# cboin1996/avddpg

Hardware: AMD Instinct MI355X
Metric: env-steps/sec + DDPG updates/sec, 4096x5-vehicle platoons (higher is better)
Workload: dtype f32-class (fp16 hi+lo operand pairs on the 16-bit matrix cores, f32 accumulate)

## Files before the change

### avddpg_amd/csrc/fsplit.hip

```cpp
#include <type_traits>

#include "fset_common.h"
#include "anchor.h"
#include "smooth.h"

namespace avd {
namespace fsplit {
using namespace fset;

struct ActorS {
    static constexpr int K = 256, KP = 256, NFT = 8, NKS = 16, LD = 264, NGT = 9, KG = 288;
    static constexpr bool critic = false;
};
struct CriticS {
    static constexpr int K = 304, KP = 320, NFT = 10, NKS = 19, LD = 312, NGT = 10, KG = 320;
    static constexpr bool critic = true;
};
constexpr int NGT_MAX = 10;

template <int I, int N, class F>
__device__ __forceinline__ void static_for(F&& f) {
    if constexpr (I < N) {
        f(std::integral_constant<int, I>{});
        static_for<I + 1, N>(f);
// ... 19 lines not shown
    f32x2 l;
#ifdef __HIP_DEVICE_COMPILE__
    asm("v_fma_mix_f32 %0, -%1, 1.0, %2 op_sel:[0,0,0] op_sel_hi:[1,0,0]" : "=v"(l[0]) : "v"(hi), "v"(a));
    asm("v_fma_mix_f32 %0, -%1, 1.0, %2 op_sel:[1,0,0] op_sel_hi:[1,0,0]" : "=v"(l[1]) : "v"(hi), "v"(b));
#else
    l[0] = a - (float)h[0], l[1] = b - (float)h[1];
#endif
    lo = __builtin_bit_cast(unsigned, __builtin_convertvector(l, f16x2));
}
__device__ __forceinline__ void split1h(float x, f16& hi, f16& lo) {
    hi = (f16)x;
    lo = (f16)(x - (float)hi);
}
template <class V>
__device__ __forceinline__ void pin16(V& x) {
#pragma unroll
    for (int q = 0; q < 2; ++q) {
        float a = x[8 * q], b = x[8 * q + 1], c = x[8 * q + 2], d = x[8 * q + 3], e = x[8 * q + 4], f = x[8 * q + 5], g = x[8 * q + 6], h = x[8 * q + 7];
        asm volatile("" : "+v"(a), "+v"(b), "+v"(c), "+v"(d), "+v"(e), "+v"(f), "+v"(g), "+v"(h));
        x[8 * q] = a, x[8 * q + 1] = b, x[8 * q + 2] = c, x[8 * q + 3] = d, x[8 * q + 4] = e, x[8 * q + 5] = f, x[8 * q + 6] = g, x[8 * q + 7] = h;
    }
}
__device__ __forceinline__ f16x8 fragh(unsigned a, unsigned b, unsigned c, unsigned d) {
    uint4 o;
    o.x = a, o.y = b, o.z = c, o.w = d;
    return __builtin_bit_cast(f16x8, o);
}
__device__ __forceinline__ f32x16 mfmah(f16x8 a, f16x8 b, f32x16 c) {
    return __builtin_amdgcn_mfma_f32_32x32x16_f16(a, b, c, 0, 0, 0);
}
__device__ __forceinline__ f16x8 make_xh(float x0, float x1, float x2, float x3, int h) {
    f16 a0, a1, a2, a3, l0, l1, l2, l3;
    split1h(x0, a0, l0), split1h(x1, a1, l1), split1h(x2, a2, l2), split1h(x3, a3, l3);
    const f16 one = (f16)1.f, zero = (f16)0.f;
    f16x8 v;
    v[0] = a0, v[1] = a1, v[2] = a2, v[3] = a3;
    v[4] = h ? one : l0, v[5] = h ? one : l1, v[6] = h ? zero : l2, v[7] = h ? zero : l3;
    return v;
}
__device__ __forceinline__ f16x8 make_wh(float w0, float w1, float w2, float w3, float b, float sc, int h) {
    f16 a0, a1, a2, a3, l0, l1, l2, l3, bh, bl;
    split1h(sc * w0, a0, l0), split1h(sc * w1, a1, l1), split1h(sc * w2, a2, l2), split1h(sc * w3, a3, l3), split1h(sc * b, bh, bl);
    const f16 zero = (f16)0.f;
    f16x8 v;
    v[0] = h ? l0 : a0, v[1] = h ? l1 : a1, v[2] = h ? l2 : a2, v[3] = h ? l3 : a3;
    v[4] = h ? bh : a0, v[5] = h ? bl : a1, v[6] = h ? bh : a2, v[7] = h ? zero : a3;
    return v;
}
__device__ __forceinline__ f16x8 make_xg(float x0, float x1, float x2, float x3, float g, int h) {
    f16 a0, a1, a2, a3, l0, l1, l2, l3, gh, gl;
    split1h(x0, a0, l0), split1h(x1, a1, l1), split1h(x2, a2, l2), split1h(x3, a3, l3), split1h(g, gh, gl);
    const f16 zero = (f16)0.f;
    f16x8 v;
    v[0] = a0, v[1] = a1, v[2] = a2, v[3] = a3;
    v[4] = h ? gh : l0, v[5] = h ? gh : l1, v[6] = h ? gl : l2, v[7] = h ? zero : l3;
    return v;
}

template <int S>
__device__ __forceinline__ void load_x(const float* xa, long row, float (&x)[4]) {
    if (S == 4) {
        const float4 v = *(const float4*)(xa + 4 * row);
        x[0] = v.x, x[1] = v.y, x[2] = v.z, x[3] = v.w;
    } else {
#pragma unroll
        for (int k = 0; k < 4; ++k) x[k] = k < S ? xa[S * row + k] : 0.f;
    }
}

__host__ __device__ constexpr int wpos(int f) { return (f & ~12) | ((f & 4) << 1) | ((f & 8) >> 1); }

struct NetP {
    const float* th;
    long th_stride;
    const f16* Whi;
    const f16* Wlo;
    const f16* Wchi;
    const f16* Wclo;
    const f16x8* wf1h;
    const float* vec;
    const unsigned* wap;
};

struct PackArgs {
    const float* x[2];
    const float* extra[2];
    f16x8* outh[2];
    long rows;
};
__device__ __forceinline__ void front_flag(unsigned* wave_flags, bool hit) {
    const bool any = __ballot(hit) != 0;
    if ((threadIdx.x & 63) == 0) wave_flags[threadIdx.x >> 6] = any;
}
template <int S>
__device__ __forceinline__ void pack_x_role(const PackArgs& a, int which, long bx, unsigned* wave_flags) {
    const float* x = a.x[which];
    const float* extra = a.extra[which];
    const bool extra_is_action = which == 0;
    const long i = bx * 256 + threadIdx.x;
    bool nf = false;
    if (i < 2 * a.rows) {
        float v[4];
        load_x<S>(x, i >> 1, v);
        nf = not_finite(v[0]) || not_finite(v[1]) || not_finite(v[2]) || not_finite(v[3]);
        nf = nf || fmaxf(fmaxf(fabsf(v[0]), fabsf(v[1])), fmaxf(fabsf(v[2]), fabsf(v[3]))) >= F16_OVERFLOW;
        if (!(i & 1)) {
            const float e = extra[i >> 1];
            nf = nf || not_finite(e) || (extra_is_action && fabsf(e) >= F16_OVERFLOW);
        }
        a.outh[which][i] = make_xh(v[0], v[1], v[2], v[3], (int)(i & 1));
    }
    front_flag(wave_flags, nf);
}

struct PrepArgs {
    avd_mlp_layout L;
    int S;
    const float *theta, *stats, *theta_t, *stats_t;
    f16 *Whi[4], *Wlo[4];
    f16 *Wchi[4], *Wclo[4];
    f16x8* wf1h[4];
    float* vec[4];
    unsigned* wap;
    unsigned* smax;
    int* bad;
    unsigned* fflag;
    int n_fflag;
};
constexpr int SCALE_SLICES = 16;
__device__ __forceinline__ float pow2_for(float mx) {
    int e = 0;
    if (mx > 0.f && !not_finite(mx)) (void)frexpf(mx, &e);
    int k = 13 - e;
    k = k < -14 ? -14 : (k > 30 ? 30 : k);
    return ldexpf(1.f, k);
}
__device__ __forceinline__ void scale_role(const PrepArgs& a, int net, int set, int slice, int n_sets) {
    __shared__ float red[256], red2[256], c3a[H2], inva[CriticS::K];
    const int tid = threadIdx.x;
    const bool critic = net & 1, target = net >= 2;
    const avd_mlp_layout& L = a.L;
    const float* th = (target ? a.theta_t : a.theta) + (long)set * L.theta_size + (critic ? L.actor_size : 0);
    const float* st = (target ? a.stats_t : a.stats) + (long)set * L.stats_size;
    const int K = critic ? CriticS::K : ActorS::K, oW2 = critic ? L.cW2 : L.aW2;
    const int og2 = critic ? L.cg3 : L.ag2, omv2 = critic ? L.cmv3 : L.amv2, oW3 = critic ? L.cW3 : L.aW3;
    if (tid < H2) c3a[tid] = fabsf((1.0f / sqrtf(st[omv2 + tid] + BN_EPS)) * th[og2 + tid] * th[oW3 + tid]);
    for (int f = tid; f < K; f += 256) {
        int og, omv, ff = f;
        if (!critic) og = L.ag1, omv = L.amv1;
        else if (f < H1) og = L.cgs, omv = L.cmvs;
        else og = L.cga, omv = L.cmva, ff = f - H1;
        inva[f] = fabsf((1.0f / sqrtf(st[omv + ff] + BN_EPS)) * th[og + ff]);
    }
    __syncthreads();
    const int total = K * H2, per = (total + SCALE_SLICES - 1) / SCALE_SLICES, lo = slice * per, hi = min(total, lo + per);
    float m = 0.f, m2 = 0.f;
    for (int i = lo + tid; i < hi; i += 256) {
        const float w = fabsf(th[oW2 + i]);
        m = fmaxf(m, inva[i / H2] * w);
        m2 = fmaxf(m2, c3a[i % H2] * w);
    }
    red[tid] = m, red2[tid] = m2;
    __syncthreads();
    for (int o = 128; o > 0; o >>= 1) {
        if (tid < o) red[tid] = fmaxf(red[tid], red[tid + o]), red2[tid] = fmaxf(red2[tid], red2[tid + o]);
        __syncthreads();
    }
    if (tid == 0) {
        unsigned* dst = a.smax + (((long)net * n_sets + set) * SCALE_SLICES + slice) * 2;
        dst[0] = __float_as_uint(red[0]);
        dst[1] = __float_as_uint(red2[0]);
    }
}
__global__ __launch_bounds__(320) void prep_kernel(const PrepArgs a) {
    __shared__ float red[320];
    const int n = blockIdx.x, net = blockIdx.y, set = blockIdx.z, f = threadIdx.x;
    const bool critic = net & 1, target = net >= 2;
    const avd_mlp_layout& L = a.L;
    const float* th = (target ? a.theta_t : a.theta) + (long)set * L.theta_size + (critic ? L.actor_size : 0);
    const float* st = (target ? a.stats_t : a.stats) + (long)set * L.stats_size;
    const int K = critic ? CriticS::K : ActorS::K, KP = critic ? CriticS::KP : ActorS::KP;
    const int oW2 = critic ? L.cW2 : L.aW2, ob2 = critic ? L.cb2 : L.ab2, oW3 = critic ? L.cW3 : L.aW3, ob3 = critic ? L.cb3 : L.ab3;
    const int og2 = critic ? L.cg3 : L.ag2, obe2 = critic ? L.cbe3 : L.abe2, omm2 = critic ? L.cmm3 : L.amm2, omv2 = critic ? L.cmv3 : L.amv2;
    const float inv2n = (1.0f / sqrtf(st[omv2 + n] + BN_EPS)) * th[og2 + n], c3n = inv2n * th[oW3 + n];
    const unsigned* smax = a.smax + ((long)net * gridDim.z + set) * SCALE_SLICES * 2;
    unsigned mx = 0, mxc = 0;
#pragma unroll
    for (int sl = 0; sl < SCALE_SLICES; ++sl) mx = max(mx, smax[2 * sl]), mxc = max(mxc, smax[2 * sl + 1]);
    const float SW = pow2_for(__uint_as_float(mx)), SWC = pow2_for(__uint_as_float(mxc));
    if (net == 0 && set == 0) {
        unsigned any = 0;
        for (int w0 = n * 320 + f; w0 < a.n_fflag; w0 += 4 * H2 * 320) {
            unsigned v[4];
#pragma unroll
            for (int u = 0; u < 4; ++u) v[u] = a.fflag[min(w0 + u * H2 * 320, a.n_fflag - 1)];
// ... 23 lines not shown
            a.Whi[net][at] = hi, a.Wlo[net][at] = lo;
        }
        if (!target) {
            f16 hi, lo;
            const float wc = SWC * (c3n * w);
            if (fabsf(wc) >= F16_OVERFLOW) atomicOr(a.bad, 1);
            split1h(wc, hi, lo);
            const long at = ((long)set * KP + f) * H2 + n;
            a.Wchi[net][at] = hi, a.Wclo[net][at] = lo;
        }
    }
    red[f] = shw;
    __syncthreads();
    if (f < 64) red[f] += red[f + 256];
    __syncthreads();
    for (int o = 128; o > 0; o >>= 1) {
        if (f < o) red[f] += red[f + o];
        __syncthreads();
    }
    float* vec = a.vec[net] + (long)set * VEC;
    if (f == 0) {
        if (n == 0) vec[2 * H2 + 1] = SW, vec[2 * H2 + 2] = SWC;
        vec[n] = th[ob2 + n] + red[0];
        vec[H2 + n] = c3n;
        if (not_finite(vec[n]) || not_finite(c3n) || not_finite(th[ob3])) atomicOr(a.bad, 1);
    }
    if (n == 0) {
        __syncthreads();
        float v = 0.f;
        if (f < H2) {
            const float inv2 = (1.0f / sqrtf(st[omv2 + f] + BN_EPS)) * th[og2 + f];
            v = (th[obe2 + f] - st[omm2 + f] * inv2) * th[oW3 + f];
        }
        red[f] = v;
        __syncthreads();
        for (int o = 64; o > 0; o >>= 1) {
            if (f < o) red[f] += red[f + o];
            __syncthreads();
        }
        if (f == 0) vec[2 * H2] = th[ob3] + red[0];
    }
}
__device__ __forceinline__ bool prep1_role(const PrepArgs& a, int ft, int net, int set, int lane) {
    const int r = lane & 31, h = lane >> 5;
    bool hit = false;
    const bool critic = net & 1, target = net >= 2;
    const avd_mlp_layout& L = a.L;
    const float* th = (target ? a.theta_t : a.theta) + (long)set * L.theta_size + (critic ? L.actor_size : 0);
    const int K = critic ? CriticS::K : ActorS::K;
    const int f = 32 * ft + r;
    float w[4] = {0.f, 0.f, 0.f, 0.f}, b = 0.f;
    if (f == K) {
        b = 1.f;
    } else if (f < K) {
        if (critic && ft >= 8) {
            w[0] = th[L.cWa + (f - H1)], b = th[L.cba + (f - H1)];
        } else {
            const float* W = th + (critic ? L.cWs : L.aW1);
#pragma unroll
            for (int k = 0; k < 4; ++k) w[k] = k < a.S ? W[k * H1 + f] : 0.f;
            b = th[(critic ? L.cbs : L.ab1) + f];
        }
        if (not_finite(w[0]) || not_finite(w[1]) || not_finite(w[2]) || not_finite(w[3]) || not_finite(b)) hit = true;
        if (S1 * fmaxf(fmaxf(fabsf(w[0]), fabsf(w[1])), fmaxf(fmaxf(fabsf(w[2]), fabsf(w[3])), fabsf(b))) >= F16_OVERFLOW) hit = true;
    }
    a.wf1h[net][((long)set * NGT_MAX + ft) * 64 + lane] = make_wh(w[0], w[1], w[2], w[3], b, S1, h);
    if (net == 1 && ft == 0 && lane < 48) {
        const int hl = lane / 24, hh = (lane / 12) & 1, ks = (lane / 4) % 3, m = lane & 3;
        unsigned v = 0;
#pragma unroll
        for (int e = 0; e < 2; ++e) {
            const int jj = 2 * m + e, fa = 16 * ks + 8 * (jj >> 2) + 4 * hh + (jj & 3);
            f16 hi, lo;
            split1h(S1 * th[L.cWa + fa], hi, lo);
            v |= (unsigned)__builtin_bit_cast(unsigned short, hl ? lo : hi) << (16 * e);
        }
        a.wap[(long)set * 48 + lane] = v;
    }
    return hit;
}

struct FrontArgs {
    PrepArgs pa;
    PackArgs pk;
    float* grads;
    long n_grads;
    int n_sets, n_scale, n_prep1, n_zero, n_pack;
};
constexpr int ZERO_PER_BLOCK = 4096;
template <int S>
__global__ __launch_bounds__(256) void front_kernel(const FrontArgs a) {
    int b = blockIdx.x;
    if (b < a.n_scale) {
        scale_role(a.pa, b & 3, (b >> 2) % a.n_sets, (b >> 2) / a.n_sets, a.n_sets);
        return;
    }
    b -= a.n_scale;
    if (b < a.n_prep1) {
        const int q = 4 * b + (threadIdx.x >> 6);
        bool hit = false;
        if (q < NGT_MAX * 4 * a.n_sets) hit = prep1_role(a.pa, q % NGT_MAX, (q / NGT_MAX) & 3, q / (NGT_MAX * 4), threadIdx.x & 63);
        front_flag(a.pa.fflag + 4 * (long)b, hit);
        return;
    }
    b -= a.n_prep1;
    if (b < a.n_zero) {
        if (b == 0 && threadIdx.x == 0) *a.pa.bad = 0;
        const long base = (long)b * ZERO_PER_BLOCK + threadIdx.x;
#pragma unroll
        for (int k = 0; k < ZERO_PER_BLOCK / 256; ++k)
            if (base + 256 * k < a.n_grads) a.grads[base + 256 * k] = 0.f;
        return;
    }
    b -= a.n_zero;
    const int which = b >= a.n_pack;
    pack_x_role<S>(a.pk, which, b - which * a.n_pack, a.pa.fflag + 4 * ((long)a.n_prep1 + b));
}

enum HeadMode { OUT_TANH = 0, OUT_TD = 1, HEAD_BOTH = 5, OUT_TANH_SAVE = 6 };
struct HeadArgs {
    unsigned long long* stamp;
    NetP net;
    int n_agents, n_sets;
    const f16x8* xf;
    const float* act;
    const float* act2;
    const float* r;
    const float* yin;
    const float* aw;
    float* out;
    unsigned* sm;
    float* g3;
    float* dmu;
    float* part_s;
    float* part_s2;
    float* part_m;
    float* tz;
    float gamma, high, inv_n;
    int* bad;
    int abl;
};
#ifndef HEAD_FAST
#define HEAD_FAST 5
#define HEAD_SLOW 3
#endif

template <int S, class NET, int MODE, bool HP = false, class... H>
__global__ __launch_bounds__(NT) void head_kernel(const HeadArgs p, H... hp) {
    constexpr int K = NET::K, NKS = NET::NKS, NFT = NET::NFT, LD = NET::LD;
    constexpr int NTH = NT;
    constexpr bool BOTH = (MODE == HEAD_BOTH);
    static_assert(!BOTH || NET::critic, "HEAD_BOTH is a critic mode");
    __shared__ __attribute__((aligned(16))) f16 wimg[2][H2 * LD];
    __shared__ __attribute__((aligned(16))) float b2s[H2];
    __shared__ __attribute__((aligned(16))) float c3s[H2];
    __shared__ __attribute__((aligned(16))) unsigned waps[BOTH ? 48 : 4];
    const int tid = threadIdx.x, w = tid >> 6, lane = tid & 63, r = lane & 31, h = lane >> 5, q = w >> 1, rh = w & 1;
    const int set = blockIdx.x % p.n_sets, j0 = blockIdx.x / p.n_sets, J = gridDim.x / p.n_sets, P = p.n_agents / p.n_sets;
#ifdef AVD_STAMP
    unsigned long long hacc[4] = {0, 0, 0, 0}, hlast = __builtin_amdgcn_s_memtime();
    const unsigned long long hstart = hlast;
#define HSTAMP(i) { const unsigned long long t_ = __builtin_amdgcn_s_memtime(); hacc[i] += t_ - hlast; hlast = t_; }
#else
#define HSTAMP(i)
#endif
    const float* vec = p.net.vec + (long)set * VEC;
    const f16x8* wf1 = p.net.wf1h + (long)set * NGT_MAX * 64 + lane;
    const f32x16 zero16 = {};
    const int ntile = j0 < P ? (P - j0 + J - 1) / J : 0;
    const int row = 32 * rh + r;
    f16x8 nx = {};
    float na = 0.f, nb = 0.f, ny = 0.f, nw = 1.f;
    auto fetch_in = [&](int k) {
        const int agent = (j0 + k * J) * p.n_sets + set;
        const long ri = (long)agent * TILE + row;
        nx = p.xf[2 * ri + h];
        if (NET::critic) na = p.act[ri];
        if (BOTH) nb = p.act2[ri];
        if (MODE == OUT_TD) ny = p.r[ri];
        if (BOTH) ny = p.yin[ri];
        if (BOTH && p.aw) nw = p.aw[agent];
    };
    constexpr int FAST = HEAD_FAST, SLOW = HEAD_SLOW, PERIOD = 2 * (FAST + SLOW);
    const int qs = __builtin_amdgcn_readfirstlane(q);
    const int cnt = qs < 2 ? FAST : SLOW, start = qs < 2 ? qs * FAST : 2 * FAST + (qs - 2) * SLOW;
    int k = start, pos = 0;
    auto next_tile = [&](int kk, int pp) { return pp + 1 == cnt ? kk + PERIOD - cnt + 1 : kk + 1; };
    const float SW = vec[2 * H2 + 1], d3 = vec[2 * H2];
    const float vb = vec[tid & (H2 - 1)], vc = vec[H2 + (tid & (H2 - 1))];
    unsigned wv = 0;
    if constexpr (BOTH) wv = p.net.wap[(long)set * 48 + (tid < 48 ? tid : 47)];
    f16x8 warm0 = wf1[0], warm1 = wf1[64];
    if (k < ntile) fetch_in(k);
    constexpr int PER = H2 * (K / 8), NLD = 2 * PER / NTH;
    static_assert(2 * PER % NTH == 0, "the image is a whole number of chunks per thread");
    typedef unsigned u32x4 __attribute__((ext_vector_type(4)));
    u32x4 img[NLD];
    static_for<0, NLD>([&](auto u_c) {
        constexpr int u = decltype(u_c)::value;
        const int i = tid + u * NTH, hl = i / PER, rem = i - hl * PER;
        img[u] = *(const u32x4*)((hl ? p.net.Wlo : p.net.Whi) + (long)set * H2 * K + 8 * rem);
    });
    __builtin_amdgcn_sched_barrier(0);
    const float sc = SW * S1, isc = 1.f / sc;
    if (tid < H2) b2s[tid] = vb * sc, c3s[tid] = vc * isc;
    if (BOTH && tid < 48) waps[tid] = wv;
    static_for<0, NLD>([&](auto u_c) {
        constexpr int u = decltype(u_c)::value;
        const int i = tid + u * NTH, hl = i / PER, rem = i - hl * PER, n = rem / (K / 8), c = rem - n * (K / 8);
        *(u32x4*)(&wimg[hl][n * LD + 8 * c]) = img[u];
    });
    asm volatile("" ::"v"(warm0), "v"(warm1));
    float Dacc = 0.f, Lacc = 0.f, Dacc2 = 0.f, Lacc2 = 0.f, gmax = 0.f;
    unsigned watch = 0;
    auto look = [&](float x) {
        unsigned u = __float_as_uint(x);
        asm volatile("" : "+v"(u));
        u &= 0x7fffffffu;
        watch = watch > u ? watch : u;
    };
    __syncthreads();

    const f16* whi0 = &wimg[0][r * LD + 8 * h];
    const f16* wlo0 = &wimg[1][r * LD + 8 * h];
    constexpr int NSEQ = BOTH ? 8 : NFT;
    HSTAMP(3);
    for (int ui = 0; k < ntile; ++ui, k = next_tile(k, pos), pos = pos + 1 == cnt ? 0 : pos + 1) {
        const int agent = (j0 + k * J) * p.n_sets + set;
        const long ri = (long)agent * TILE + row;
        const f16x8 xs = nx, xa = make_xh(na, 0.f, 0.f, 0.f, h), xb = BOTH ? make_xh(nb, 0.f, 0.f, 0.f, h) : xa;
        const float ty = ny, tw = nw;
        if (next_tile(k, pos) < ntile) fetch_in(next_tile(k, pos));
        f32x16 acc[4];
#pragma unroll
        for (int t = 0; t < 4; ++t)
#pragma unroll
            for (int g = 0; g < 4; ++g) {
                const float4 b = *(const float4*)(b2s + 32 * t + 8 * g + 4 * h);
                acc[t][4 * g] = b.x, acc[t][4 * g + 1] = b.y, acc[t][4 * g + 2] = b.z, acc[t][4 * g + 3] = b.w;
            }
        unsigned ph[8], pl[8];
        auto split16 = [&](const f32x16& p1) {
            if (FSPLIT_ABL(p.abl) & 4) {
#pragma unroll
                for (int m = 0; m < 8; ++m) ph[m] = __float_as_uint(p1[2 * m]), pl[m] = __float_as_uint(p1[2 * m + 1]);
                return;
            }
#pragma unroll
            for (int m = 0; m < 8; ++m) split2h(relu(p1[2 * m]), relu(p1[2 * m + 1]), ph[m], pl[m]);
        };
        auto zdot_t = [&](f32x16& a, int t) {
            float zp = 0.f;
#pragma unroll
            for (int g = 0; g < 4; ++g) {
                const float4 c = *(const float4*)(c3s + 32 * t + 8 * g + 4 * h);
                const float cc[4] = {c.x, c.y, c.z, c.w};
#pragma unroll
                for (int j = 0; j < 4; ++j) {
                    a[4 * g + j] = relu(a[4 * g + j]);
                    zp = fmaf(a[4 * g + j], cc[j], zp);
                }
            }
            return zp;
        };
        auto zdot_nd = [&](const f32x16& a, int t) {
            float zp = 0.f;
#pragma unroll
            for (int g = 0; g < 4; ++g) {
                const float4 c = *(const float4*)(c3s + 32 * t + 8 * g + 4 * h);
                const float cc[4] = {c.x, c.y, c.z, c.w};
#pragma unroll
                for (int j = 0; j < 4; ++j) zp = fmaf(relu(a[4 * g + j]), cc[j], zp);
            }
            return zp;
        };
        auto mask_t = [&](const f32x16& a) {
            unsigned b = 0;
#pragma unroll
            for (int g = 0; g < 4; ++g)
#pragma unroll
                for (int j = 0; j < 4; ++j) b |= a[4 * g + j] > 0.f ? 1u << (4 * g + (j >> 1) + 16 * (j & 1)) : 0u;
            return b;
        };
        auto mask_store = [&](const unsigned (&b)[4], unsigned* dst) {
            const auto s0 = __builtin_amdgcn_permlane32_swap(b[0], b[2], false, false);
            const auto s1 = __builtin_amdgcn_permlane32_swap(b[1], b[3], false, false);
            uint2 o;
            o.x = s0[0] | (s0[1] << 2), o.y = s1[0] | (s1[1] << 2);
            *(uint2*)(dst + 2 * h) = o;
        };
        auto out_z = [&](f32x16 (&ac)[4]) {
            float zp = 0.f;
#pragma unroll
            for (int t = 0; t < 4; ++t) zp += zdot_t(ac[t], t);
            zp += __shfl_xor(zp, 32);
            return d3 + zp;
        };
        split16(mfmah(wf1[0], xs, zero16));
        f16x8 wfn = wf1[64];
        f16x8 wg[2][2][2];
        auto read_group = [&](int g, f16x8 (&dst)[2][2]) {
            const int ks = g >> 1, th = g & 1;
#pragma unroll
            for (int tt = 0; tt < 2; ++tt) {
                dst[tt][0] = *(const f16x8*)(whi0 + 32 * (2 * th + tt) * LD + 16 * ks);
                dst[tt][1] = *(const f16x8*)(wlo0 + 32 * (2 * th + tt) * LD + 16 * ks);
            }
        };
        read_group(0, wg[0]);
        auto tile = [&](auto si_c, f32x16 (&ac)[4]) {
            constexpr int si = decltype(si_c)::value;
            constexpr int ft = si;
            f32x16 p1n = zero16;
            if constexpr (si + 1 < NSEQ) {
                p1n = mfmah(wfn, (NET::critic && si + 1 >= 8) ? xa : xs, zero16);
                if constexpr (si + 2 < NSEQ) wfn = wf1[64 * (si + 2)];
            }
#pragma unroll
            for (int s = 0; s < 2; ++s) {
                const int ks = 2 * ft + s;
                if (ks >= NKS) continue;
                const f16x8 bhi = fragh(ph[4 * s], ph[4 * s + 1], ph[4 * s + 2], ph[4 * s + 3]);
                const f16x8 blo = fragh(pl[4 * s], pl[4 * s + 1], pl[4 * s + 2], pl[4 * s + 3]);
#pragma unroll
                for (int th = 0; th < 2; ++th) {
                    const int g = 2 * ks + th;
                    if (g + 1 < 2 * (BOTH ? 16 : NKS)) read_group(g + 1, wg[(g + 1) & 1]);
#pragma unroll
                    for (int tt = 0; tt < 2; ++tt) {
                        const int t = 2 * th + tt;
                        const f16x8 whi = wg[g & 1][tt][0], wlo = wg[g & 1][tt][1];
                        ac[t] = mfmah(whi, bhi, ac[t]);
                        ac[t] = mfmah(wlo, bhi, ac[t]);
                        ac[t] = mfmah(whi, blo, ac[t]);
                    }
                }
            }
            if constexpr (si + 1 < NSEQ) split16(p1n);
            __builtin_amdgcn_sched_group_barrier(0x008, 1, 0);
#pragma unroll
            for (int gi = 0; gi < 4; ++gi) {
                __builtin_amdgcn_sched_group_barrier(0x100, 4, 0);
#pragma unroll
                for (int i = 0; i < 6; ++i) {
                    __builtin_amdgcn_sched_group_barrier(0x008, 1, 0);
                    __builtin_amdgcn_sched_group_barrier(0x002, 3, 0);
                }
            }
            __builtin_amdgcn_sched_barrier(0);
        };
        HSTAMP(0);
        static_for<0, NSEQ>([&](auto si_c) { tile(si_c, acc); });
        HSTAMP(1);
        if constexpr (BOTH) {
            f16x8 fh[3], fl[3];
            auto act_sweep = [&](f32x16 (&c)[4]) {
                f16x8 wq[2][2][2];
                read_group(2 * 16, wq[0]);
#pragma unroll
                for (int g = 0; g < 6; ++g) {
                    if (g + 1 < 6) read_group(2 * 16 + g + 1, wq[(g + 1) & 1]);
#pragma unroll
                    for (int tt = 0; tt < 2; ++tt) {
                        const int t = 2 * (g & 1) + tt;
                        const f16x8 whi = wq[g & 1][tt][0], wlo = wq[g & 1][tt][1];
                        c[t] = mfmah(whi, fh[g >> 1], c[t]);
                        c[t] = mfmah(wlo, fh[g >> 1], c[t]);
                        c[t] = mfmah(whi, fl[g >> 1], c[t]);
                    }
                }
            };
#pragma unroll
            for (int tl = 0; tl < 2; ++tl) {
                const f32x16 p1 = mfmah(wf1[64 * (8 + tl)], xa, zero16);
                split16(p1);
#pragma unroll
                for (int ss = 0; ss < 2 - tl; ++ss) {
                    fh[2 * tl + ss] = fragh(ph[4 * ss], ph[4 * ss + 1], ph[4 * ss + 2], ph[4 * ss + 3]);
                    fl[2 * tl + ss] = fragh(pl[4 * ss], pl[4 * ss + 1], pl[4 * ss + 2], pl[4 * ss + 3]);
                }
            }
            act_sweep(acc);
            look(acc[0][0]);
            {
                float zp = 0.f;
#pragma unroll
                for (int t = 0; t < 4; ++t) zp += zdot_nd(acc[t], t);
                zp += __shfl_xor(zp, 32);
                const float diff = d3 + zp - ty, g3a = 2.f * diff * p.inv_n * tw;
                if (h == 0) p.g3[ri] = g3a, Dacc += g3a, Lacc += diff * diff;
                gmax = fmaxf(gmax, fabsf(g3a));
                unsigned mb[4];
#pragma unroll
                for (int t = 0; t < 4; ++t) mb[t] = mask_t(acc[t]);
                mask_store(mb, p.sm + ri * 4);
            }
            __builtin_amdgcn_sched_barrier(0);
            f16x8 mh[3], ml[3];
#pragma unroll
            for (int tl = 0; tl < 2; ++tl) {
                const f32x16 pa = mfmah(wf1[64 * (8 + tl)], xa, zero16), pm = mfmah(wf1[64 * (8 + tl)], xb, zero16);
                unsigned dh[8], dl[8], mk[8];
#pragma unroll
                for (int m = 0; m < 4 * (2 - tl); ++m) {
                    split2h(relu(pm[2 * m]) - relu(pa[2 * m]), relu(pm[2 * m + 1]) - relu(pa[2 * m + 1]), dh[m], dl[m]);
                    mk[m] = (pm[2 * m] > 0.f ? 0xffffu : 0u) | (pm[2 * m + 1] > 0.f ? 0xffff0000u : 0u);
                }
#pragma unroll
                for (int ss = 0; ss < 2 - tl; ++ss) {
                    const int kk = 2 * tl + ss;
                    fh[kk] = fragh(dh[4 * ss], dh[4 * ss + 1], dh[4 * ss + 2], dh[4 * ss + 3]);
                    fl[kk] = fragh(dl[4 * ss], dl[4 * ss + 1], dl[4 * ss + 2], dl[4 * ss + 3]);
                    const uint4 ch = *(const uint4*)(waps + (0 * 2 + h) * 12 + 4 * kk), cl = *(const uint4*)(waps + (1 * 2 + h) * 12 + 4 * kk);
                    mh[kk] = fragh(ch.x & mk[4 * ss], ch.y & mk[4 * ss + 1], ch.z & mk[4 * ss + 2], ch.w & mk[4 * ss + 3]);
                    ml[kk] = fragh(cl.x & mk[4 * ss], cl.y & mk[4 * ss + 1], cl.z & mk[4 * ss + 2], cl.w & mk[4 * ss + 3]);
                }
            }
            act_sweep(acc);
            look(acc[0][0]);
            float zq = 0.f;
            unsigned pos[2] = {0u, 0u};
// ... 590 lines not shown
    const float wa = f < HA ? th[p.L_cWa + f] : 0.f, ba = f < HA ? th[p.L_cba + f] : 0.f;
    float Sa = 0.f, Sb = 0.f;
    const int ntile = j0 < P ? (P - j0 + J - 1) / J : 0;
    uint4 mA = {}, mB = {};
    float gA = 0.f, aA = 0.f, gB = 0.f, aB = 0.f;
#define DXA_FETCH(k_, m_, g_, a_)                                                                                   \
    {                                                                                                               \
        const long r0_ = (long)((j0 + (k_) * J) * p.n_sets + set) * TILE + 32 * rh;                                 \
        m_ = *(const uint4*)(p.sm + (r0_ + r) * 4);                                                                 \
        g_ = p.g3[r0_ + r], a_ = p.act[r0_ + r];                                                                    \
    }
#define DXA_PUT(buf_, g_, a_)                                                                                       \
    {                                                                                                               \
        if (h == 0) ga[w][buf_][0][r] = fabsf(g_) * gv, ga[w][buf_][1][r] = a_;                                     \
        __builtin_amdgcn_fence(__ATOMIC_RELEASE, "wavefront");                                                      \
        __builtin_amdgcn_wave_barrier();                                                                            \
    }
    auto unit = [&](int buf, const uint4 mw, float g) {
        f32x16 dc = zero16;
        const unsigned m = mask_one(g, true);
        const unsigned mwt[4] = {mw.x >> (4 * h), mw.y >> (4 * h), mw.z >> (4 * h), mw.w >> (4 * h)};
#pragma unroll
        for (int s = 0; s < 8; ++s) {
            const unsigned d = mwt[s >> 1] >> (8 * (s & 1));
            const f16x8 af = fragh(mask_pair(d, 0, m), mask_pair(d, 1, m >> 1), mask_pair(d, 2, m >> 2), mask_pair(d, 3, m >> 3));
            dc = mfmah(af, wch[s], dc), dc = mfmah(af, wcl[s], dc);
        }
        float sa = 0.f, sb = 0.f;
#pragma unroll
        for (int q = 0; q < 4; ++q) {
            const float4 gq = *(const float4*)(&ga[w][buf][0][8 * q + 4 * h]), aq = *(const float4*)(&ga[w][buf][1][8 * q + 4 * h]);
            const float gg[4] = {gq.x, gq.y, gq.z, gq.w}, av[4] = {aq.x, aq.y, aq.z, aq.w};
#pragma unroll
            for (int j = 0; j < 4; ++j) {
                const float m = fmaf(av[j], wa, ba) > 0.f ? dc[4 * q + j] * gg[j] : 0.f;
                sa = fmaf(m, av[j], sa);
                sb += m;
            }
        }
        Sa += sa, Sb += sb;
        __builtin_amdgcn_fence(__ATOMIC_ACQ_REL, "wavefront");
        __builtin_amdgcn_wave_barrier();
    };
    if (par < ntile) DXA_FETCH(par, mA, gA, aA);
    if (par + 2 < ntile) DXA_FETCH(par + 2, mB, gB, aB);
    const float gsc = set_gscale(p.part_m, set, p.n_sets, J, gred);
    const float gv = gsc * VSH, vs = gsc * swc * VSH;
    for (int k = par; k < ntile; k += 4) {
        DXA_PUT(0, gA, aA);
        {
            const uint4 mc = mA;
            const float gc = gA;
            if (k + 4 < ntile) DXA_FETCH(k + 4, mA, gA, aA);
            unit(0, mc, gc);
        }
        if (k + 2 < ntile) {
            DXA_PUT(1, gB, aB);
            const uint4 mc = mB;
            const float gc = gB;
            if (k + 6 < ntile) DXA_FETCH(k + 6, mB, gB, aB);
            unit(1, mc, gc);
        }
    }
#undef DXA_FETCH
#undef DXA_PUT
    comb[w][lane][0] = Sa, comb[w][lane][1] = Sb;
    __syncthreads();
    if (rh == 0 && par == 0 && h == 0) {
        const int ws[4] = {w, w + 1, w + 4, w + 5};
        float t[2] = {0.f, 0.f};
#pragma unroll
        for (int i = 0; i < 4; ++i)
#pragma unroll
            for (int c = 0; c < 2; ++c) t[c] += comb[ws[i]][r][c] + comb[ws[i]][32 + r][c];
        const float ivs = 1.f / vs;
        float* pv = p.partV + ((long)blockIdx.x * KP + 32 * ft + r) * 16;
#pragma unroll
        for (int c = 0; c < 9; ++c) pv[c] = c == 0 ? t[0] * ivs : (c == 8 ? t[1] * ivs : 0.f);
    }
}

struct Plan {
    int grid, J;
    size_t Whi[4], Wlo[4], Wchi[2], Wclo[2], wf1h[4], vec[4], wap, a2, y, mu, dmu, g3, sm, sma, tz, t1p, s2raw, xfs, xfs2, partHs[3], partM[2],
        partV[2], partG[2], bad, smax, fflag, total;
    int n_prep1, n_pack, n_fflag;
};
static Plan make_plan(int n_agents, int n_sets) {
    Plan pl;
    const int P = n_agents / n_sets;
    int J = cu_count() / n_sets;
    if (const char* e = AVD_DIAG_ENV("FSPLIT_J")) J = atoi(e);
    if (J < 1) J = 1;
    if (J > P) J = P;
    pl.J = J, pl.grid = J * n_sets;
    size_t o = 0;
    auto take = [&](size_t bytes) {
        const size_t at = o;
        o += (bytes + 255) / 256 * 256;
        return at;
    };
    for (int i = 0; i < 4; ++i) {
        const int K = (i & 1) ? CriticS::K : ActorS::K, KP = (i & 1) ? CriticS::KP : ActorS::KP;
        pl.Whi[i] = take(sizeof(f16) * (size_t)n_sets * H2 * K), pl.Wlo[i] = take(sizeof(f16) * (size_t)n_sets * H2 * K);
        pl.vec[i] = take(sizeof(float) * (size_t)n_sets * VEC);
        pl.wf1h[i] = take(16 * (size_t)n_sets * NGT_MAX * 64);
        if (i < 2) pl.Wchi[i] = take(sizeof(f16) * (size_t)n_sets * KP * H2), pl.Wclo[i] = take(sizeof(f16) * (size_t)n_sets * KP * H2);
    }
    pl.wap = take(4 * (size_t)n_sets * 48);
    const size_t rows = (size_t)n_agents * TILE;
    pl.a2 = take(4 * rows), pl.y = take(4 * rows), pl.mu = take(4 * rows), pl.dmu = take(4 * rows), pl.g3 = take(4 * rows);
    pl.sm = take(16 * rows);
    pl.sma = take(16 * rows);
    pl.tz = take(4 * rows);
    pl.t1p = take(2 * 4 * (size_t)n_sets * CriticS::K * H2), pl.s2raw = take(2 * 4 * (size_t)n_sets * H2);
    pl.xfs = take(32 * rows), pl.xfs2 = take(32 * rows);
    for (int i = 0; i < 2; ++i) {
        const int KP = i ? CriticS::KP : ActorS::KP, KG = i ? CriticS::KG : ActorS::KG;
        pl.partM[i] = take(4 * (size_t)pl.grid * 8);
        pl.partV[i] = take(4 * (size_t)pl.grid * KP * 16);
        pl.partG[i] = take(4 * (size_t)pl.grid * KG * H2);
    }
    for (int i = 0; i < 3; ++i) pl.partHs[i] = take(4 * (size_t)pl.grid * 8 * 2);
    pl.n_prep1 = (NGT_MAX * 4 * n_sets + 3) / 4, pl.n_pack = (int)((2 * rows + 255) / 256);
    pl.n_fflag = 4 * (pl.n_prep1 + 2 * pl.n_pack);
    pl.bad = take(sizeof(int));
    pl.smax = take(sizeof(unsigned) * 4 * (size_t)n_sets * SCALE_SLICES * 2);
    pl.fflag = take(sizeof(unsigned) * (size_t)pl.n_fflag);
    pl.total = o;
    return pl;
}
static int check_shape(const avd_mlp_layout* L, int n_agents, int n_sets, const char* who) {
    AVD_REQUIRE(L, "%s: null layout", who);
    if (L->H1 != H1 || L->H2 != H2 || L->Ha != HA || L->A != 1 || (L->S != 3 && L->S != 4) || L->B != TILE) {
        set_error("%s: serves the reference widths only (layer1 256, layer2 128, action layer 48, A = 1, S in {3, 4}, B = 64); "
                  "got H1=%d H2=%d Ha=%d A=%d S=%d B=%d (avd_learn_shared_bf16 takes other widths)",
                  who, L->H1, L->H2, L->Ha, L->A, L->S, L->B);
        return AVD_E_UNSUPPORTED;
    }
    AVD_REQUIRE(n_sets > 0 && n_sets <= 64 && n_agents > 0 && n_agents % n_sets == 0, "%s: n_agents=%d n_sets=%d", who, n_agents,
                n_sets);
    return AVD_OK;
}

enum Phase { PH_CRITIC = 1, PH_ACTOR = 2, PH_BOTH = 3 };
#ifdef AVD_STAMP
static unsigned long long* head_stamps() {
    static unsigned long long* m = nullptr;
    if (!m && hipHostMalloc(&m, 4 * 128 * 8, hipHostMallocDefault) == hipSuccess) memset(m, 0, 4 * 128 * 8);
    return m;
}
static void print_head_stamps(hipStream_t st) {
    (void)hipStreamSynchronize(st);
    static const char* who[4] = {"actor OUT_TANH_SAVE", "critic HEAD_BOTH", "target actor OUT_TANH", "target critic OUT_TD"};
    for (int ni = 0; ni < 4; ++ni)
        for (int w = 0; w < 8; ++w) {
            const unsigned long long* s = head_stamps() + 128 * ni + 8 * w;
            fprintf(stderr, "HSTAMP %-22s wave %d: start-up %8llu  unit-start %8llu  tiles %9llu  epilogue %8llu  start-up share %.4f\n", who[ni], w,
                    s[3], s[0], s[1], s[2], (double)s[3] / (double)(s[0] + s[1] + s[2] + s[3] + 1));
        }
}
#endif
template <int S, class... H>
static int run(int phases, const avd_mlp_layout& L, int n_agents, int n_sets, const float* theta, const float* stats, const float* theta_t,
               const float* stats_t, const float* s, const float* a, const float* r, const float* s2, const float* aw, float gamma,
               float high, float* grads, float* losses, unsigned char* ws, const Plan& pl, hipStream_t st, const AnchorArgs* an,
               const SmoothArgs* smo, H... hp) {
    PrepArgs pa;
    pa.L = L, pa.S = S, pa.theta = theta, pa.stats = stats, pa.theta_t = theta_t, pa.stats_t = stats_t;
    pa.wap = (unsigned*)(ws + pl.wap), pa.bad = (int*)(ws + pl.bad), pa.smax = (unsigned*)(ws + pl.smax);
    pa.fflag = (unsigned*)(ws + pl.fflag), pa.n_fflag = pl.n_fflag;
    NetP net[4];
    for (int i = 0; i < 4; ++i) {
        const bool critic = i & 1, target = i >= 2;
        pa.Whi[i] = (f16*)(ws + pl.Whi[i]), pa.Wlo[i] = (f16*)(ws + pl.Wlo[i]), pa.vec[i] = (float*)(ws + pl.vec[i]);
        pa.wf1h[i] = (f16x8*)(ws + pl.wf1h[i]);
        pa.Wchi[i] = i < 2 ? (f16*)(ws + pl.Wchi[i]) : nullptr, pa.Wclo[i] = i < 2 ? (f16*)(ws + pl.Wclo[i]) : nullptr;
        NetP& n = net[i];
        n.th = (target ? theta_t : theta) + (critic ? L.actor_size : 0), n.th_stride = L.theta_size;
        n.Whi = pa.Whi[i], n.Wlo = pa.Wlo[i], n.Wchi = pa.Wchi[i], n.Wclo = pa.Wclo[i], n.wf1h = pa.wf1h[i], n.vec = pa.vec[i];
        n.wap = pa.wap;
    }
    const int P = n_agents / n_sets;
    const float inv_n = 1.0f / ((float)P * TILE);
    const long nrows = (long)n_agents * TILE;
    f16x8 *xfs = (f16x8*)(ws + pl.xfs), *xfs2 = (f16x8*)(ws + pl.xfs2);
    int* bad = (int*)(ws + pl.bad);
    float *a2 = (float*)(ws + pl.a2), *y = (float*)(ws + pl.y), *mu = (float*)(ws + pl.mu), *dmu = (float*)(ws + pl.dmu);
    float* g3 = (float*)(ws + pl.g3);
    unsigned *sm = (unsigned*)(ws + pl.sm), *sma = (unsigned*)(ws + pl.sma);
    auto F = [&](size_t off) { return (float*)(ws + off); };
    const dim3 grid(pl.grid), block(NT);
    HeadArgs h;
    h.n_agents = n_agents, h.n_sets = n_sets, h.gamma = gamma, h.high = high, h.inv_n = inv_n, h.aw = aw, h.sm = sm, h.g3 = g3, h.dmu = dmu;
    h.act2 = nullptr, h.part_s2 = nullptr, h.stamp = nullptr, h.bad = bad, h.part_m = nullptr, h.tz = F(pl.tz), h.abl = 0;
    if (const char* e = AVD_DIAG_ENV("FSPLIT_ABL")) h.abl = atoi(e);
    auto head = [&](auto kern, int ni, const f16x8* x, const float* act, const float* rr, const float* yin, float* out, float* part_s,
                    auto... extra) {
        h.net = net[ni], h.xf = x, h.act = act, h.r = rr, h.yin = yin, h.out = out, h.part_s = part_s;
#ifdef AVD_STAMP
        h.stamp = head_stamps() + 128 * ni;
#endif
        hipLaunchKernelGGL(kern, grid, block, 0, st, h, extra...);
    };
    DwArgs dw;
    dw.n_agents = n_agents, dw.n_sets = n_sets, dw.sm = sm, dw.g3 = g3, dw.x = s, dw.stamp = nullptr, dw.abl = 0;
    if (const char* e = AVD_DIAG_ENV("FSPLIT_ABL")) dw.abl = atoi(e);
#ifdef AVD_STAMP
    static unsigned long long* d_stamp = nullptr;
    if (!d_stamp) (void)hipMalloc(&d_stamp, 128 * 8);
    dw.stamp = d_stamp;
#endif
    DxArgs dx;
    dx.n_agents = n_agents, dx.n_sets = n_sets, dx.sm = sm, dx.g3 = g3, dx.xfh = xfs, dx.stamp = nullptr, dx.L_cWa = dx.L_cba = 0;
    dx.abl = dw.abl;
#ifdef AVD_STAMP
    dx.stamp = d_stamp;
#endif
    FinArgs fa;
    fa.L = L, fa.n_sets = n_sets, fa.J = pl.J, fa.S = S, fa.nrh = 1, fa.theta = theta, fa.stats = stats, fa.grads = grads, fa.losses = losses;
    fa.inv_n = inv_n, fa.partLa = F(pl.partHs[2]), fa.bad = bad;
    for (int i = 0; i < 2; ++i)
        fa.partH[i] = nullptr, fa.partHs[i] = F(pl.partHs[i]), fa.partU[i] = nullptr, fa.partV[i] = F(pl.partV[i]),
        fa.partG[i] = F(pl.partG[i]), fa.c3[i] = F(pl.vec[i]);
    fa.t1_from_g[0] = fa.t1_from_g[1] = 1, fa.t1p = F(pl.t1p), fa.s2raw = F(pl.s2raw);
    if (phases & PH_CRITIC) {
        FrontArgs fr;
        fr.pa = pa, fr.grads = grads, fr.n_grads = (long)n_sets * L.theta_size, fr.n_sets = n_sets;
        fr.pk.x[0] = s, fr.pk.extra[0] = a, fr.pk.outh[0] = xfs, fr.pk.x[1] = s2, fr.pk.extra[1] = r, fr.pk.outh[1] = xfs2, fr.pk.rows = nrows;
        fr.n_scale = 4 * n_sets * SCALE_SLICES, fr.n_prep1 = pl.n_prep1, fr.n_pack = pl.n_pack;
        fr.n_zero = (int)((fr.n_grads + ZERO_PER_BLOCK - 1) / ZERO_PER_BLOCK);
        hipLaunchKernelGGL(front_kernel<S>, dim3((unsigned)(fr.n_scale + fr.n_prep1 + fr.n_zero + 2 * fr.n_pack)), dim3(256), 0, st, fr);
        hipLaunchKernelGGL(prep_kernel, dim3(H2, 4, n_sets), dim3(320), 0, st, pa);
        head(head_kernel<S, ActorS, OUT_TANH>, 2, xfs2, nullptr, nullptr, nullptr, a2, nullptr);
        if (smo) {
            SmoothArgs q = *smo;
            q.n_agents = n_agents, q.a2 = a2;
            launch_target_smooth(q, st);
        }
        if constexpr (sizeof...(H) > 0)
            head(head_kernel<S, CriticS, OUT_TD, true, H...>, 3, xfs2, a2, r, nullptr, y, nullptr, hp...);
        else
            head(head_kernel<S, CriticS, OUT_TD>, 3, xfs2, a2, r, nullptr, y, nullptr);
        h.sm = sma;
        head(head_kernel<S, ActorS, OUT_TANH_SAVE>, 0, xfs, nullptr, nullptr, nullptr, mu, nullptr);
        h.sm = sm;
        h.act2 = mu, h.part_s2 = F(pl.partHs[2]), h.part_m = F(pl.partM[1]);
        head(head_kernel<S, CriticS, HEAD_BOTH>, 1, xfs, a, nullptr, y, nullptr, F(pl.partHs[1]));
        dw.net = net[1], dw.act = a, dw.partG = F(pl.partG[1]), dw.part_m = F(pl.partM[1]);
        hipLaunchKernelGGL((dw_kernel<S, CriticS>), grid, block, 0, st, dw);
        dx.net = net[1], dx.partV = F(pl.partV[1]), dx.act = a, dx.part_m = F(pl.partM[1]);
        hipLaunchKernelGGL((dx_kernel<S, CriticS>), grid, block, 0, st, dx);
        dx.L_cWa = L.cWa, dx.L_cba = L.cba;
        hipLaunchKernelGGL((dxa_kernel<S>), grid, block, 0, st, dx);
        if (phases == PH_CRITIC) launch_finalize(fa, st, 1, 1);
    }
    if (phases & PH_ACTOR) {
        SeedArgs sd;
        sd.n_agents = n_agents, sd.n_sets = n_sets, sd.dmu = dmu, sd.tz = F(pl.tz), sd.high = high, sd.g3 = g3, sd.part_m = F(pl.partM[0]),
        sd.part_s = F(pl.partHs[0]);
        if (an) {
            AnchorArgs q = *an;
            q.n_agents = n_agents, q.n_sets = n_sets, q.S = S, q.J = pl.J, q.dmu = dmu, q.tz = sd.tz, q.high = high, q.g3 = g3;
            q.part_m = sd.part_m, q.part_s = sd.part_s, q.mu = mu, q.s = s, q.aw = aw, q.inv_n = inv_n, q.c = 2.f * an->weight * inv_n;
            q.bad = bad;
            launch_anchor_seed(q, pl.grid, st);
        } else
            hipLaunchKernelGGL(actor_seed_kernel, grid, block, 0, st, sd);
        dw.sm = sma, dx.sm = sma;
        dw.net = net[0], dw.act = nullptr, dw.partG = F(pl.partG[0]), dw.part_m = F(pl.partM[0]);
        hipLaunchKernelGGL((dw_kernel<S, ActorS>), grid, block, 0, st, dw);
        dx.net = net[0], dx.partV = F(pl.partV[0]), dx.act = nullptr, dx.part_m = F(pl.partM[0]), dx.L_cWa = dx.L_cba = 0;
        hipLaunchKernelGGL((dx_kernel<S, ActorS>), grid, block, 0, st, dx);
        if (phases == PH_ACTOR) launch_finalize(fa, st, 0, 1);
        else launch_finalize(fa, st, 0, 2);
    }
#ifdef AVD_STAMP
    if (AVD_DIAG_ENV("FSPLIT_STAMPS")) print_head_stamps(st);
#endif
    return check_launch("avd_learn_set_split");
}

}
}

using namespace avd;

namespace avd { namespace fsplit {
constexpr long MFMA_PER_TILE = 2 * (200 + 238 + 200 + 314)
                               + 8 * (2 + 32 + 1 + 2 * 2 * 2)
                               + 8 * (2 + 32 + 1 + 2 * 1 * 2)
                               + 2 * 8 * (32 + 2 + 8)
                               + 4 * 16;
static_assert(MFMA_PER_TILE == 3296, "update DESIGN.md 3.4 and the count above together");
}}
extern "C" int avd_learn_set_split_mfma_count(const avd_mlp_layout* lay, int n_agents, int n_sets, unsigned long long* mfma_32x32x16) {
    int rc = fsplit::check_shape(lay, n_agents, n_sets, "avd_learn_set_split_mfma_count");
    if (rc) return rc;
    AVD_REQUIRE(mfma_32x32x16, "avd_learn_set_split_mfma_count: null pointer");
    *mfma_32x32x16 = (unsigned long long)fsplit::MFMA_PER_TILE * (unsigned long long)n_agents;
    return AVD_OK;
}

extern "C" int avd_learn_set_split_workspace(const avd_mlp_layout* lay, int n_agents, int n_sets, size_t* bytes) {
    int rc = fsplit::check_shape(lay, n_agents, n_sets, "avd_learn_set_split_workspace");
    if (rc) return rc;
    AVD_REQUIRE(bytes, "avd_learn_set_split_workspace: null pointer");
    *bytes = fsplit::make_plan(n_agents, n_sets).total;
    return AVD_OK;
}

template <class... H>
static int split_entry(int phases, const char* who, const avd_mlp_layout* lay, int n_agents, int n_sets, const float* theta, const float* stats,
                       const float* theta_t, const float* stats_t, const float* s, const float* a, const float* r, const float* s2,
                       const float* agent_weight, float gamma, float high, float* grads, float* losses, void* workspace,
                       size_t workspace_bytes, void* stream, const AnchorArgs* an, const SmoothArgs* smo, H... hp) {
    int rc = fsplit::check_shape(lay, n_agents, n_sets, who);
    if (rc) return rc;
    const bool cr = phases & fsplit::PH_CRITIC;
    AVD_REQUIRE(theta && stats && s && grads && workspace && (!cr || (theta_t && stats_t && a && r && s2)), "%s: null pointer", who);
    const fsplit::Plan pl = fsplit::make_plan(n_agents, n_sets);
    AVD_REQUIRE(workspace_bytes >= pl.total, "%s: workspace %zu B < %zu B", who, workspace_bytes, pl.total);
    if (lay->S == 4)
        return fsplit::run<4>(phases, *lay, n_agents, n_sets, theta, stats, theta_t, stats_t, s, a, r, s2, agent_weight, gamma, high, grads,
                              losses, (unsigned char*)workspace, pl, (hipStream_t)stream, an, smo, hp...);
    return fsplit::run<3>(phases, *lay, n_agents, n_sets, theta, stats, theta_t, stats_t, s, a, r, s2, agent_weight, gamma, high, grads, losses,
                          (unsigned char*)workspace, pl, (hipStream_t)stream, an, smo, hp...);
}

extern "C" int avd_learn_set_split_f16x3(const avd_mlp_layout* lay, int n_agents, int n_sets, const float* theta, const float* stats,
                                          const float* theta_t, const float* stats_t, const float* s, const float* a, const float* r,
// ... 93 lines not shown
```

Baseline: 2.218 million.

## Fuse input packing into head kernels, dropping separate pack pass and buffer

Removes the pack role from the front kernel, which converted raw state rows into fp16 hi/lo pairs and checked them for non-finite or overflow values. The non-BOTH head kernels now load raw f32 states directly, convert them in-register, and fold the finiteness and range checks into their existing watch logic. The actor-save head writes the packed image for the later critic HEAD_BOTH pass. This drops one full read/write pass over the inputs and the xfs2 buffer, but adds conversion and check work inside the heads' latency-hidden prefetch path. It also moves the input validation from front flags into the heads' own watch mechanism.

Result: no change. 2.240 million, median of 6 (+1.0%).

```diff
diff --git a/avddpg_amd/csrc/fsplit.hip b/avddpg_amd/csrc/fsplit.hip
--- a/avddpg_amd/csrc/fsplit.hip
+++ b/avddpg_amd/csrc/fsplit.hip
@@ -125,35 +125,9 @@
     const unsigned* wap;
 };
 
-struct PackArgs {
-    const float* x[2];
-    const float* extra[2];
-    f16x8* outh[2];
-    long rows;
-};
 __device__ __forceinline__ void front_flag(unsigned* wave_flags, bool hit) {
     const bool any = __ballot(hit) != 0;
     if ((threadIdx.x & 63) == 0) wave_flags[threadIdx.x >> 6] = any;
-}
-template <int S>
-__device__ __forceinline__ void pack_x_role(const PackArgs& a, int which, long bx, unsigned* wave_flags) {
-    const float* x = a.x[which];
-    const float* extra = a.extra[which];
-    const bool extra_is_action = which == 0;
-    const long i = bx * 256 + threadIdx.x;
-    bool nf = false;
-    if (i < 2 * a.rows) {
-        float v[4];
-        load_x<S>(x, i >> 1, v);
-        nf = not_finite(v[0]) || not_finite(v[1]) || not_finite(v[2]) || not_finite(v[3]);
-        nf = nf || fmaxf(fmaxf(fabsf(v[0]), fabsf(v[1])), fmaxf(fabsf(v[2]), fabsf(v[3]))) >= F16_OVERFLOW;
-        if (!(i & 1)) {
-            const float e = extra[i >> 1];
-            nf = nf || not_finite(e) || (extra_is_action && fabsf(e) >= F16_OVERFLOW);
-        }
-        a.outh[which][i] = make_xh(v[0], v[1], v[2], v[3], (int)(i & 1));
-    }
-    front_flag(wave_flags, nf);
 }
 
 struct PrepArgs {
@@ -343,13 +317,11 @@
 
 struct FrontArgs {
     PrepArgs pa;
-    PackArgs pk;
     float* grads;
     long n_grads;
-    int n_sets, n_scale, n_prep1, n_zero, n_pack;
+    int n_sets, n_scale, n_prep1, n_zero;
 };
 constexpr int ZERO_PER_BLOCK = 4096;
-template <int S>
 __global__ __launch_bounds__(256) void front_kernel(const FrontArgs a) {
     int b = blockIdx.x;
     if (b < a.n_scale) {
@@ -365,17 +337,11 @@
         return;
     }
     b -= a.n_prep1;
-    if (b < a.n_zero) {
-        if (b == 0 && threadIdx.x == 0) *a.pa.bad = 0;
-        const long base = (long)b * ZERO_PER_BLOCK + threadIdx.x;
-#pragma unroll
-        for (int k = 0; k < ZERO_PER_BLOCK / 256; ++k)
-            if (base + 256 * k < a.n_grads) a.grads[base + 256 * k] = 0.f;
-        return;
-    }
-    b -= a.n_zero;
-    const int which = b >= a.n_pack;
-    pack_x_role<S>(a.pk, which, b - which * a.n_pack, a.pa.fflag + 4 * ((long)a.n_prep1 + b));
+    if (b == 0 && threadIdx.x == 0) *a.pa.bad = 0;
+    const long base = (long)b * ZERO_PER_BLOCK + threadIdx.x;
+#pragma unroll
+    for (int k = 0; k < ZERO_PER_BLOCK / 256; ++k)
+        if (base + 256 * k < a.n_grads) a.grads[base + 256 * k] = 0.f;
 }
 
 enum HeadMode { OUT_TANH = 0, OUT_TD = 1, HEAD_BOTH = 5, OUT_TANH_SAVE = 6 };
@@ -400,6 +366,8 @@
     float gamma, high, inv_n;
     int* bad;
     int abl;
+    const float* xraw;
+    f16x8* xsave;
 };
 #ifndef HEAD_FAST
 #define HEAD_FAST 5
@@ -430,13 +398,16 @@
     const f32x16 zero16 = {};
     const int ntile = j0 < P ? (P - j0 + J - 1) / J : 0;
     const int row = 32 * rh + r;
+    constexpr bool RAW = !BOTH;
     f16x8 nx = {};
+    float nxr[4] = {0.f, 0.f, 0.f, 0.f};
     float na = 0.f, nb = 0.f, ny = 0.f, nw = 1.f;
     auto fetch_in = [&](int k) {
         const int agent = (j0 + k * J) * p.n_sets + set;
         const long ri = (long)agent * TILE + row;
-        nx = p.xf[2 * ri + h];
-        if (NET::critic) na = p.act[ri];
+        if constexpr (RAW) load_x<S>(p.xraw, ri, nxr);
+        else nx = p.xf[2 * ri + h];
+        if (NET::critic || MODE == OUT_TANH_SAVE) na = p.act[ri];
         if (BOTH) nb = p.act2[ri];
         if (MODE == OUT_TD) ny = p.r[ri];
         if (BOTH) ny = p.yin[ri];
@@ -480,6 +451,25 @@
         u &= 0x7fffffffu;
         watch = watch > u ? watch : u;
     };
+    auto look_in = [&](const float* x, int n, bool range) {
+        unsigned m = 0;
+#pragma unroll
+        for (int i = 0; i < n; ++i) {
+            unsigned u = __float_as_uint(x[i]);
+            asm("" : "+v"(u));
+            u &= 0x7fffffffu;
+            m = m > u ? m : u;
+        }
+        const unsigned hit = range ? (m >= __builtin_bit_cast(unsigned, F16_OVERFLOW) ? 0x7f800000u : 0u) : m;
+        watch = watch > hit ? watch : hit;
+    };
+    auto take_in = [&]() {
+        nx = make_xh(nxr[0], nxr[1], nxr[2], nxr[3], h);
+        if (MODE == OUT_TANH || MODE == OUT_TANH_SAVE) look_in(nxr, S, true);
+        if (MODE == OUT_TANH_SAVE) look_in(&na, 1, true);
+        if (MODE == OUT_TD) look_in(&ny, 1, false);
+    };
+    if constexpr (RAW) take_in();
     __syncthreads();
 
     const f16* whi0 = &wimg[0][r * LD + 8 * h];
@@ -490,6 +480,7 @@
         const int agent = (j0 + k * J) * p.n_sets + set;
         const long ri = (long)agent * TILE + row;
         const f16x8 xs = nx, xa = make_xh(na, 0.f, 0.f, 0.f, h), xb = BOTH ? make_xh(nb, 0.f, 0.f, 0.f, h) : xa;
+        if (MODE == OUT_TANH_SAVE) p.xsave[2 * ri + h] = xs;
         const float ty = ny, tw = nw;
         if (next_tile(k, pos) < ntile) fetch_in(next_tile(k, pos));
         f32x16 acc[4];
@@ -598,6 +589,7 @@
                 }
             }
             if constexpr (si + 1 < NSEQ) split16(p1n);
+            else if constexpr (RAW) take_in();
             __builtin_amdgcn_sched_group_barrier(0x008, 1, 0);
 #pragma unroll
             for (int gi = 0; gi < 4; ++gi) {
@@ -1354,9 +1346,9 @@
 
 struct Plan {
     int grid, J;
-    size_t Whi[4], Wlo[4], Wchi[2], Wclo[2], wf1h[4], vec[4], wap, a2, y, mu, dmu, g3, sm, sma, tz, t1p, s2raw, xfs, xfs2, partHs[3], partM[2],
+    size_t Whi[4], Wlo[4], Wchi[2], Wclo[2], wf1h[4], vec[4], wap, a2, y, mu, dmu, g3, sm, sma, tz, t1p, s2raw, xfs, partHs[3], partM[2],
         partV[2], partG[2], bad, smax, fflag, total;
-    int n_prep1, n_pack, n_fflag;
+    int n_prep1, n_fflag;
 };
 static Plan make_plan(int n_agents, int n_sets) {
     Plan pl;
@@ -1386,7 +1378,7 @@
     pl.sma = take(16 * rows);
     pl.tz = take(4 * rows);
     pl.t1p = take(2 * 4 * (size_t)n_sets * CriticS::K * H2), pl.s2raw = take(2 * 4 * (size_t)n_sets * H2);
-    pl.xfs = take(32 * rows), pl.xfs2 = take(32 * rows);
+    pl.xfs = take(32 * rows);
     for (int i = 0; i < 2; ++i) {
         const int KP = i ? CriticS::KP : ActorS::KP, KG = i ? CriticS::KG : ActorS::KG;
         pl.partM[i] = take(4 * (size_t)pl.grid * 8);
@@ -1394,8 +1386,8 @@
         pl.partG[i] = take(4 * (size_t)pl.grid * KG * H2);
     }
     for (int i = 0; i < 3; ++i) pl.partHs[i] = take(4 * (size_t)pl.grid * 8 * 2);
-    pl.n_prep1 = (NGT_MAX * 4 * n_sets + 3) / 4, pl.n_pack = (int)((2 * rows + 255) / 256);
-    pl.n_fflag = 4 * (pl.n_prep1 + 2 * pl.n_pack);
+    pl.n_prep1 = (NGT_MAX * 4 * n_sets + 3) / 4;
+    pl.n_fflag = 4 * pl.n_prep1;
     pl.bad = take(sizeof(int));
     pl.smax = take(sizeof(unsigned) * 4 * (size_t)n_sets * SCALE_SLICES * 2);
     pl.fflag = take(sizeof(unsigned) * (size_t)pl.n_fflag);
@@ -1455,8 +1447,7 @@
     }
     const int P = n_agents / n_sets;
     const float inv_n = 1.0f / ((float)P * TILE);
-    const long nrows = (long)n_agents * TILE;
-    f16x8 *xfs = (f16x8*)(ws + pl.xfs), *xfs2 = (f16x8*)(ws + pl.xfs2);
+    f16x8* xfs = (f16x8*)(ws + pl.xfs);
     int* bad = (int*)(ws + pl.bad);
     float *a2 = (float*)(ws + pl.a2), *y = (float*)(ws + pl.y), *mu = (float*)(ws + pl.mu), *dmu = (float*)(ws + pl.dmu);
     float* g3 = (float*)(ws + pl.g3);
@@ -1467,9 +1458,10 @@
     h.n_agents = n_agents, h.n_sets = n_sets, h.gamma = gamma, h.high = high, h.inv_n = inv_n, h.aw = aw, h.sm = sm, h.g3 = g3, h.dmu = dmu;
     h.act2 = nullptr, h.part_s2 = nullptr, h.stamp = nullptr, h.bad = bad, h.part_m = nullptr, h.tz = F(pl.tz), h.abl = 0;
     if (const char* e = AVD_DIAG_ENV("FSPLIT_ABL")) h.abl = atoi(e);
-    auto head = [&](auto kern, int ni, const f16x8* x, const float* act, const float* rr, const float* yin, float* out, float* part_s,
+    h.xf = nullptr, h.xraw = nullptr, h.xsave = nullptr;
+    auto head = [&](auto kern, int ni, const float* x, const float* act, const float* rr, const float* yin, float* out, float* part_s,
                     auto... extra) {
-        h.net = net[ni], h.xf = x, h.act = act, h.r = rr, h.yin = yin, h.out = out, h.part_s = part_s;
+        h.net = net[ni], h.xraw = x, h.act = act, h.r = rr, h.yin = yin, h.out = out, h.part_s = part_s;
 #ifdef AVD_STAMP
         h.stamp = head_stamps() + 128 * ni;
 #endif
@@ -1499,26 +1491,25 @@
     if (phases & PH_CRITIC) {
         FrontArgs fr;
         fr.pa = pa, fr.grads = grads, fr.n_grads = (long)n_sets * L.theta_size, fr.n_sets = n_sets;
-        fr.pk.x[0] = s, fr.pk.extra[0] = a, fr.pk.outh[0] = xfs, fr.pk.x[1] = s2, fr.pk.extra[1] = r, fr.pk.outh[1] = xfs2, fr.pk.rows = nrows;
-        fr.n_scale = 4 * n_sets * SCALE_SLICES, fr.n_prep1 = pl.n_prep1, fr.n_pack = pl.n_pack;
+        fr.n_scale = 4 * n_sets * SCALE_SLICES, fr.n_prep1 = pl.n_prep1;
         fr.n_zero = (int)((fr.n_grads + ZERO_PER_BLOCK - 1) / ZERO_PER_BLOCK);
-        hipLaunchKernelGGL(front_kernel<S>, dim3((unsigned)(fr.n_scale + fr.n_prep1 + fr.n_zero + 2 * fr.n_pack)), dim3(256), 0, st, fr);
+        hipLaunchKernelGGL(front_kernel, dim3((unsigned)(fr.n_scale + fr.n_prep1 + fr.n_zero)), dim3(256), 0, st, fr);
         hipLaunchKernelGGL(prep_kernel, dim3(H2, 4, n_sets), dim3(320), 0, st, pa);
-        head(head_kernel<S, ActorS, OUT_TANH>, 2, xfs2, nullptr, nullptr, nullptr, a2, nullptr);
+        head(head_kernel<S, ActorS, OUT_TANH>, 2, s2, nullptr, nullptr, nullptr, a2, nullptr);
         if (smo) {
             SmoothArgs q = *smo;
             q.n_agents = n_agents, q.a2 = a2;
             launch_target_smooth(q, st);
         }
         if constexpr (sizeof...(H) > 0)
-            head(head_kernel<S, CriticS, OUT_TD, true, H...>, 3, xfs2, a2, r, nullptr, y, nullptr, hp...);
+            head(head_kernel<S, CriticS, OUT_TD, true, H...>, 3, s2, a2, r, nullptr, y, nullptr, hp...);
         else
-            head(head_kernel<S, CriticS, OUT_TD>, 3, xfs2, a2, r, nullptr, y, nullptr);
-        h.sm = sma;
-        head(head_kernel<S, ActorS, OUT_TANH_SAVE>, 0, xfs, nullptr, nullptr, nullptr, mu, nullptr);
-        h.sm = sm;
-        h.act2 = mu, h.part_s2 = F(pl.partHs[2]), h.part_m = F(pl.partM[1]);
-        head(head_kernel<S, CriticS, HEAD_BOTH>, 1, xfs, a, nullptr, y, nullptr, F(pl.partHs[1]));
+            head(head_kernel<S, CriticS, OUT_TD>, 3, s2, a2, r, nullptr, y, nullptr);
+        h.sm = sma, h.xsave = xfs;
+        head(head_kernel<S, ActorS, OUT_TANH_SAVE>, 0, s, a, nullptr, nullptr, mu, nullptr);
+        h.sm = sm, h.xsave = nullptr;
+        h.act2 = mu, h.part_s2 = F(pl.partHs[2]), h.part_m = F(pl.partM[1]), h.xf = xfs;
+        head(head_kernel<S, CriticS, HEAD_BOTH>, 1, nullptr, a, nullptr, y, nullptr, F(pl.partHs[1]));
         dw.net = net[1], dw.act = a, dw.partG = F(pl.partG[1]), dw.part_m = F(pl.partM[1]);
         hipLaunchKernelGGL((dw_kernel<S, CriticS>), grid, block, 0, st, dw);
         dx.net = net[1], dx.partV = F(pl.partV[1]), dx.act = a, dx.part_m = F(pl.partM[1]);
```
